# jyf588/transformer-inertial-poser

Measured on AMD Instinct MI355X. Metric: IMU frames/sec (whole node), seq_len=40 batch=256/GPU, higher is better.
Workload: dtype f32

## Files before the change

### include/tip_hip.h

```cpp
#ifndef TIP_HIP_H
#define TIP_HIP_H

#include <stddef.h>
#include <stdint.h>

#ifdef __cplusplus
extern "C" {
#endif

#define TIP_ABI_VERSION 5

#define TIP_API __attribute__((visibility("default")))

typedef struct tip_handle tip_handle;
typedef void* tip_stream_t;

typedef struct tip_config {
    int32_t input_size_imu;
    int32_t size_s;
    int32_t rnn_hid_size;
    int32_t tf_hid_size;
    int32_t tf_in_dim;
    int32_t n_heads;
    int32_t tf_layers;
// ... 19 lines not shown

#define TIP_PLAN_AUTO    0
#define TIP_PLAN_GENERAL 1
#define TIP_PLAN_FUSED   2
#define TIP_PLAN_FUSED2  4
#define TIP_PLAN_FUSEDH  6
#define TIP_PLAN_LATENCY 3

#define TIP_PLAN_FUSED1S 10

#define TIP_OPT_PLAN        1
#define TIP_OPT_PROFILE     2
#define TIP_OPT_RNN_CLUSTER 3
#define TIP_RNN_CLUSTER_ROWS4 0x44
#define TIP_OPT_FAULT_INJECT 4

#define TIP_OPT_FUSE_HEAD 5

#define TIP_OPT_AUTO_DEMOTE 7
#define TIP_OPT_DEMOTED     8
#define TIP_OPT_NO_FLOW    10
#define TIP_OPT_HANDOFF_KIND 11
#define TIP_OPT_NO_ROUND_LAUNCH 12
#define TIP_OPT_F1S_PARTS   9

TIP_API int tip_abi_version(void);
TIP_API int tip_create(const tip_config* cfg, tip_handle** out);
TIP_API void tip_destroy(tip_handle* h);
TIP_API const char* tip_strerror(int status);
TIP_API const char* tip_last_hip_error(const tip_handle* h);
TIP_API int tip_set_option(tip_handle* h, int option, int value);
TIP_API int tip_get_option(const tip_handle* h, int option, int* value);

TIP_API int tip_num_tensors(const tip_handle* h);
TIP_API int tip_tensor_info(const tip_handle* h, int i, const char** name, int* rows, int* cols );
TIP_API int tip_packed_bytes(const tip_handle* h, size_t* bytes);
TIP_API int tip_pack_weights(const tip_handle* h, const float* const* host_tensors, int n, void* packed_host_out, size_t bytes);
TIP_API int tip_pack_weights_device(const tip_handle* h, const float* const* tensors, int n, void* packed_dev, size_t bytes,
                            tip_stream_t stream);
TIP_API int tip_attach_packed(tip_handle* h, const void* packed_device, size_t bytes);

TIP_API int tip_workspace_bytes(const tip_handle* h, int B, int T, size_t* bytes);
TIP_API int tip_max_batch(const tip_handle* h, int T, int fp64, int* max_batch);
TIP_API int tip_forward(tip_handle* h, const float* x_imu, const float* x_s, float* y, int B, int T, int flags,
                const float* keep_mask, float keep_scale, void* workspace, size_t workspace_bytes,
                tip_stream_t stream);
// ... 283 lines not shown
```

### transformer-inertial-poser_amd/csrc/tip_abi.hip

```cpp
#include <math.h>
#include <string.h>

#include <new>

#include <mutex>
#include "tip_internal.h"
#include <atomic>
#include <chrono>

using namespace tip;

namespace {

const char* kStatusText[] = {
    "ok",
    "invalid argument",
    "unsupported configuration",
    "not ready: no packed weights attached",
    "workspace too small or misaligned",
    "HIP runtime error",
    "no HIP device",
    "allocation failure",
    "an inter-workgroup hand-off wait gave up in an earlier launch (outputs of that launch are NaN-poisoned); tip_check(h, 1) clears",
};

size_t align_up(size_t x, size_t a) { return (x + a - 1) / a * a; }

void build_tensor_table(tip_handle* h) {
    const Dims& d = h->d;
    auto add = [&](const std::string& n, int r, int cdim) {
        h->tensor_names.push_back(n);
// ... 89 lines not shown
        stop = pr.second;
    }
    ~StageScope() {
        if (stop) (void)hipEventRecord(stop, s);
    }
};

}

static hipError_t linear_gemm(const float* P, const tip::PackedLinear& p, const float* A, int lda, const float* res, int ldres,
                              float* C, int ldc, int M, int flags, hipStream_t s) {
    auto al16 = [](const void* q, int ld) { return (reinterpret_cast<uintptr_t>(q) & 15) == 0 && (ld & 3) == 0; };
    if (p.f_off && tip::pgemm_shape_ok(M, p.N, p.K) && al16(P + p.b_off, 0) && al16(C, ldc) && (!(flags & 2) || al16(res, ldres)))
        return tip::launch_pgemm(A, lda, P + p.f_off, (size_t)p.N * p.K, P + p.b_off, res, ldres, C, ldc, M, p.N, p.K, flags, s);
    return tip::launch_gemm(A, lda, P + p.w_off, p.Kpad, P + p.b_off, res, ldres, C, ldc, M, p.N, p.Npad, flags, s);
}

namespace tip {
namespace {
struct DevSerialState {
    std::mutex mu;
    hipStream_t last = nullptr;
    bool have = false;
    hipEvent_t ev = nullptr;
};
DevSerialState g_serial[kMaxDevices];
}

CoopSerial::CoopSerial(int device, hipStream_t s)
    : dev(device >= 0 && device < kMaxDevices ? device : tip_cur_device()), stream(s), capturing(stream_is_capturing(s)), status(hipSuccess) {
    DevSerialState& st = g_serial[dev];
    st.mu.lock();
    if (capturing) return;
    if (st.have && st.last != s && st.ev) status = hipStreamWaitEvent(s, st.ev, 0);
}

CoopSerial::~CoopSerial() {
    DevSerialState& st = g_serial[dev];
    if (!capturing) {
        if (!st.ev && hipEventCreateWithFlags(&st.ev, hipEventDisableTiming) != hipSuccess) {
            (void)hipGetLastError();
            st.ev = nullptr;
        }
        if (st.ev) (void)hipEventRecord(st.ev, stream);
        st.last = stream;
        st.have = true;
    }
    st.mu.unlock();
}
}

extern "C" {

int tip_abi_version(void) { return TIP_ABI_VERSION; }

const char* tip_strerror(int status) {
    const int i = -status;
    if (i < 0 || i >= (int)(sizeof(kStatusText) / sizeof(kStatusText[0]))) return "unknown status";
    return kStatusText[i];
}

int tip_create(const tip_config* cfg, tip_handle** out) {
    if (!cfg || !out) return TIP_ERR_INVALID_ARG;
    *out = nullptr;
    Dims d{};
    d.n_imu_total = cfg->input_size_imu + (cfg->with_acc_sum ? 18 : 0);
    d.S = cfg->size_s;
    d.In = d.n_imu_total + d.S;
    d.InPad = round_up(d.In, kGemmBK);
    d.D = cfg->tf_in_dim;
    d.H = cfg->n_heads;
// ... 42 lines not shown
            if (hipHostGetDevicePointer(&dp, hp, 0) == hipSuccess && dp) {
                h->err_host = static_cast<unsigned*>(hp);
                h->err_dev = static_cast<unsigned*>(dp);
            } else {
                (void)hipHostFree(hp);
            }
        }
        (void)hipGetLastError();
    } else {
        (void)hipGetLastError();
    }
    *out = h;
    return TIP_OK;
}

void tip_destroy(tip_handle* h) {
    if (!h) return;
    for (auto& t : h->timers)
        for (auto& pr : t.pairs) {
            (void)hipEventDestroy(pr.first);
            (void)hipEventDestroy(pr.second);
        }
    if (h->err_host) (void)hipHostFree(h->err_host);
    delete h;
}

const char* tip_last_hip_error(const tip_handle* h) { return h ? h->last_hip_error.c_str() : ""; }

int tip_set_option(tip_handle* h, int option, int value) {
    if (!h) return TIP_ERR_INVALID_ARG;
    switch (option) {
        case TIP_OPT_PLAN:
            if (value < TIP_PLAN_AUTO || value > TIP_PLAN_FUSED1S || value == 9 ) return TIP_ERR_INVALID_ARG;
            if (value == 5 || value == 7 || value == 8) return TIP_ERR_UNSUPPORTED_CONFIG;
            h->plan = value;
            return TIP_OK;
        case TIP_OPT_PROFILE:
            if (value < 0 || value > 3) return TIP_ERR_INVALID_ARG;
            h->profile = value;
            for (auto& t : h->timers) t.used = 0;
            return TIP_OK;
        case TIP_OPT_RNN_CLUSTER:
            if (!(value == 0 || value == 1 || value == 2 || value == 4 || value == 8 || value == 16 || value == 32 || value == TIP_RNN_CLUSTER_ROWS4))
                return TIP_ERR_INVALID_ARG;
            h->rnn_cluster = value;
            return TIP_OK;
// ... 5 lines not shown
            if (value < 0 || value > 1) return TIP_ERR_INVALID_ARG;
            h->fuse_head = value;
            return TIP_OK;
        case TIP_OPT_AUTO_DEMOTE:
            if (value < 0 || value > 1) return TIP_ERR_INVALID_ARG;
            h->auto_demote = value;
            return TIP_OK;
        case TIP_OPT_DEMOTED:
            if (value < 0 || value > 1) return TIP_ERR_INVALID_ARG;
            h->demoted = value;
            return TIP_OK;
        case TIP_OPT_F1S_PARTS:
            if (value != 0 && value != 2 && value != 4) return TIP_ERR_INVALID_ARG;
            h->f1s_parts = value;
            return TIP_OK;
        case TIP_OPT_NO_FLOW:
            if (value < 0 || value > 1) return TIP_ERR_INVALID_ARG;
            h->no_flow = value;
            return TIP_OK;
        case TIP_OPT_NO_ROUND_LAUNCH:
            if (value < 0 || value > 1) return TIP_ERR_INVALID_ARG;
            h->no_round_launch = value;
            return TIP_OK;
        default: return TIP_ERR_INVALID_ARG;
    }
}

int tip_check(tip_handle* h, int clear) {
    if (!h) return TIP_ERR_INVALID_ARG;
    if (!h->err_host) return TIP_OK;
    volatile unsigned* w = const_cast<volatile unsigned*>(h->err_host);
    const unsigned v = w[0] | w[1];
    if (clear) w[0] = w[1] = 0u;
    return v ? TIP_ERR_HANDOFF : TIP_OK;
}

int tip_get_option(const tip_handle* h, int option, int* value) {
    if (!h || !value) return TIP_ERR_INVALID_ARG;
    switch (option) {
        case TIP_OPT_PLAN: *value = h->plan; return TIP_OK;
        case TIP_OPT_PROFILE: *value = h->profile; return TIP_OK;
        case TIP_OPT_RNN_CLUSTER: *value = h->rnn_cluster; return TIP_OK;
        case TIP_OPT_FAULT_INJECT: *value = h->fault_inject; return TIP_OK;
        case TIP_OPT_FUSE_HEAD: *value = h->fuse_head; return TIP_OK;
        case TIP_OPT_AUTO_DEMOTE: *value = h->auto_demote; return TIP_OK;
        case TIP_OPT_DEMOTED: *value = h->demoted; return TIP_OK;
        case TIP_OPT_F1S_PARTS: *value = h->f1s_parts; return TIP_OK;
        case TIP_OPT_NO_FLOW: *value = h->no_flow; return TIP_OK;
        case TIP_OPT_NO_ROUND_LAUNCH: *value = h->no_round_launch; return TIP_OK;
        case TIP_OPT_HANDOFF_KIND: {
            const volatile unsigned* w = const_cast<const volatile unsigned*>(h->err_host);
            *value = !w ? 0 : w[0] ? 1 : w[1] ? 2 : 0;
            return TIP_OK;
        }
        default: return TIP_ERR_INVALID_ARG;
    }
}

int tip_num_tensors(const tip_handle* h) { return h ? (int)h->tensor_names.size() : TIP_ERR_INVALID_ARG; }

int tip_tensor_info(const tip_handle* h, int i, const char** name, int* rows, int* cols) {
    if (!h || i < 0 || i >= (int)h->tensor_names.size()) return TIP_ERR_INVALID_ARG;
    if (name) *name = h->tensor_names[i].c_str();
    if (rows) *rows = h->tensor_shapes[i].first;
    if (cols) *cols = h->tensor_shapes[i].second;
    return TIP_OK;
}

int tip_packed_bytes(const tip_handle* h, size_t* bytes) {
    if (!h || !bytes) return TIP_ERR_INVALID_ARG;
    *bytes = h->lay.total_floats * sizeof(float);
    return TIP_OK;
// ... 104 lines not shown
    bool rnn_done = false, head_done = false;
    bool round_launch = false;
};

#define TIP_TRY(expr, what)                                     \
    do {                                                        \
        const hipError_t e_ = (expr);                           \
        if (e_ != hipSuccess) return fail_hip(q.h, e_, what);   \
    } while (0)
#define TIP_STAGE(name, expr)              \
    do {                                   \
        StageScope stage_(q.h, q.s, name); \
        TIP_TRY(expr, name);               \
    } while (0)

static int launch_round(LaunchSeq& q, const float* x_imu, const float* x_s, const float* mask, float* ih, float* hall) {
    tip_handle* h = q.h;
    const Dims& d = h->d;
    const float* P = h->packed_dev;
    const PackedLayout& L = h->lay;
    const bool last_only = (q.flags & TIP_FWD_LAST_ROW_ONLY) != 0;
    const int head = q.T == 40 && measure_switches().head_ksplit ? (last_only ? 2 : 1) : 0;
    StageScope sc(h, q.s, "fused_encoder");
    const hipError_t e = launch_forward_round(d, P + L.fused_off, x_imu, x_s, mask, q.keep_scale, ih, hall,
                                              reinterpret_cast<unsigned*>(q.W0 + q.ws.flags), P + L.whh_frag_off, P + L.out_frag_off,
                                              P + L.out_lin.b_off, q.y, q.n, q.T, head, q.cus, h->guard(), q.s);
    if (e == hipErrorCooperativeLaunchTooLarge || e == hipErrorInvalidValue) {
        (void)hipGetLastError();
        return 0;
    }
    if (e != hipSuccess) return fail_hip(h, e, "forward_round");
    q.ih_done = q.hall_armed = q.rnn_done = true;
    q.head_done = head != 0;
    return 1;
}

static int run_encoder(LaunchSeq& q, const SchedPart& p, int off) {
    tip_handle* h = q.h;
    const Dims& d = h->d;
    const float* P = h->packed_dev;
    const PackedLayout& L = h->lay;
    hipStream_t s = q.s;
    const int B = p.count, T = q.T, cus = q.cus, M = B * T;
    const size_t row_i = (size_t)T * d.n_imu_total, row_s = (size_t)T * d.S, row_r = (size_t)T * d.R;
    const float* x_imu = q.x_imu + off * row_i;
    const float* x_s = q.x_s + off * row_s;
    const float* mask = q.mask ? q.mask + off * row_s : nullptr;
    const float keep_scale = q.keep_scale;
    float* xa = q.W0 + q.ws.xa;
// ... 289 lines not shown
```

### transformer-inertial-poser_amd/csrc/tip_fused_h.h

```cpp
#pragma once
#include "tip_internal.h"
#include "tip_attention.h"
#include "tip_layernorm.h"

namespace tip {

typedef float f32x4 __attribute__((ext_vector_type(4)));

namespace fz {
constexpr int D = 256, H = 16, DH = 16, F = 1024, RP = 48, RB = 3, TMAX = 40, R = 512;
constexpr int KIN = 224;
constexpr int LDX = D + 8;
constexpr int LDC = 128 + 4;
constexpr int LDV = RP + 4;
constexpr int LDU = KIN + 8;
constexpr int X_FLOATS = RP * LDX;
constexpr int C_FLOATS = 2 * RP * LDC + 128 * LDV;
constexpr int LDS_BYTES = (X_FLOATS + C_FLOATS) * 4;
constexpr int THREADS = 512;
constexpr size_t IN_W = 0;
constexpr size_t IN_B = IN_W + (size_t)D * KIN;
constexpr size_t LAYER0 = IN_B + D;
constexpr size_t QKV_W = 0;
constexpr size_t QKV_B = QKV_W + (size_t)3 * D * D;
// ... 201 lines not shown
}

__device__ __forceinline__ f32x4 tail_gather_v(const f32x4& a0, const f32x4& a1, int lg) {
    f32x4 o;
#pragma unroll
    for (int e = 0; e < 4; ++e) {
        float x = a0[e], y = a1[e];
        swap16(x, y);
        float s = x + y, t = s;
        swap32(s, t);
        o[e] = s + t;
    }
    return lg < 2 ? o : (f32x4){0.f, 0.f, 0.f, 0.f};
}

extern __device__ unsigned long long g_fh_trace[64];
extern __device__ unsigned long long g_fh_wg[2 * 1024];
#define FH_STAMP(slot) do { if (TRACE && blockIdx.x == 0 && tid == 0 && (layer == 1 || (slot) < 4 || (slot) >= 40)) g_fh_trace[slot] = __builtin_amdgcn_s_memtime(); } while (0)

struct FhGridStride {
    static constexpr int kAux = 0;
    __device__ __forceinline__ int first() const { return blockIdx.x; }
    __device__ __forceinline__ int stride() const { return gridDim.x; }
    __device__ __forceinline__ void published(int, int) const {}
};

template <bool TRACE, bool TR, bool LIVE, class Ctl>
__device__ __forceinline__ void fused_encoder_h_body(
    const float* __restrict__ wts, const float* __restrict__ x_imu, const float* __restrict__ x_s, const float* __restrict__ keep_mask, float keep_scale, float* __restrict__ xout, float* __restrict__ ih_out,
    unsigned* __restrict__ hall_sentinel, int B, int T, int NI, int S, int L, int wbytes, int ih_off_b, const FusedEncArgs<LIVE>& tr, Ctl ctl) {
#include "tip_fused_h_body.inc"
}

}
```

### transformer-inertial-poser_amd/csrc/tip_fused_h_body.inc

```
    using namespace fz;
    using namespace fzh;
    extern __shared__ __attribute__((aligned(16))) float smem[];
    float* X = smem;
    float* C = smem + X_FLOATS;
    const int tid = threadIdx.x, lane = tid & 63;
    const int wave = __builtin_amdgcn_readfirstlane(tid >> 6);
    const int l15 = lane & 15, lg = lane >> 4;
    const __amdgpu_buffer_rsrc_t rsrc = __builtin_amdgcn_make_buffer_rsrc(const_cast<float*>(wts), 0, wbytes, 0x00020000);
    const int voff = lane * 16;
    auto am = [&](int ld) { return l15 * ld + lg * 4; };
    auto at = [&](int ld) { return (TAIL0 + (lane & 3)) * ld + lg * 4; };
    constexpr bool DR = TR || LIVE;
    const LiveArgs lv = live_args_of(tr);
    unsigned long long dseed = tr.seed, sseed = 0;
    if (LIVE) {
        sseed = lv.state_seed;
        if (lv.seeds) { dseed = lv.seeds[0]; sseed = lv.seeds[1]; }
    }
    const unsigned mkey = LIVE && lv.mthresh ? tip_drop_key_s(sseed, kStateMaskSite) : 0u;

    for (int i = tid; i < 8 * LDX; i += THREADS) X[TMAX * LDX + i] = 0.f;

    for (int win = ctl.first(); win < B; win += ctl.stride()) {
        WRing<3> g_qkv;
// ... 319 lines not shown
            const int lo = opaque(lane), l15o = lo & 15, lgo = lo >> 4;
            float bvs[4];
            f32x4 bv4s[4];
#pragma unroll
            for (int n = 0; n < 4; ++n) {
                bvs[n] = wts[ih_off_b / 4 + R * D + (wave * 4 + n) * 16 + l15o];
                bv4s[n] = *reinterpret_cast<const f32x4*>(wts + ih_off_b / 4 + R * D + (wave * 4 + n) * 16 + lgo * 4);
            }
#pragma unroll
            for (int n = 0; n < 4; ++n) {
                const int col = (wave * 4 + n) * 16 + l15o;
#pragma unroll
                for (int r = 0; r < RBM; ++r) {
                    const int row = r * 16 + l15o;
                    __builtin_amdgcn_raw_buffer_store_b128(__builtin_bit_cast(u32x4, acc[r][n] + bv4s[n]), io_rs, (row * R + (wave * 4 + n) * 16 + lgo * 4) * 4, 0, Ctl::kAux);
                }
#pragma unroll
                for (int r = 0; r < RBT; ++r) {
                    const float v = tail_reduce(acct[r][n], lg) + bvs[n];
                    const int row = TAIL0 + 4 * r + lgo;
                    __builtin_amdgcn_raw_buffer_store_b32(__float_as_uint(v), io_rs, (row * R + col) * 4, 0, Ctl::kAux);
                }
            }
        }
        if (hall_sentinel) {
            if constexpr (Ctl::kAux != 0) {
                const __amdgpu_buffer_rsrc_t hs_rs = __builtin_amdgcn_make_buffer_rsrc(hall_sentinel + (size_t)win * T * R, 0, T * R * 4, 0x00020000);
                const u32x4 ones = {0xFFFFFFFFu, 0xFFFFFFFFu, 0xFFFFFFFFu, 0xFFFFFFFFu};
                for (int i = opaque(tid); i < T * (R / 4); i += THREADS) __builtin_amdgcn_raw_buffer_store_b128(ones, hs_rs, i * 16, 0, Ctl::kAux);
            } else {
            uint4* hp = reinterpret_cast<uint4*>(hall_sentinel + (size_t)win * T * R);
            for (int i = opaque(tid); i < T * (R / 4); i += THREADS) hp[i] = make_uint4(0xFFFFFFFFu, 0xFFFFFFFFu, 0xFFFFFFFFu, 0xFFFFFFFFu);
            }
        }
        if (xout) {
            float* out = xout + (size_t)win * T * D;
            for (int i = tid; i < T * (D / 4); i += THREADS) {
                const int r = i / (D / 4), c4 = i - r * (D / 4);
                *reinterpret_cast<float4*>(out + (size_t)r * D + c4 * 4) = *reinterpret_cast<const float4*>(X + r * LDX + c4 * 4);
            }
        }
        __syncthreads();
        { const int layer = -1; FH_STAMP(41); }
        if (TRACE && tid == 0 && blockIdx.x < 1024) g_fh_wg[2 * blockIdx.x + 1] = __builtin_amdgcn_s_memrealtime();
        ctl.published(win, tid);
    }
// ... 1 lines not shown
```

### transformer-inertial-poser_amd/csrc/tip_rnn_rows4.h

```cpp
#pragma once
#include "tip_internal.h"
#include "tip_layernorm.h"

namespace tip {

typedef float f32x4 __attribute__((ext_vector_type(4)));
typedef unsigned int u32x4 __attribute__((ext_vector_type(4)));

constexpr unsigned kRnnSentinel = 0xFFFFFFFFu;
constexpr int kQ4Rows = 4, kQ4Cluster = 4, kQ4Tiles = 4, kQ4LD = 512 + 16;

struct RnnFromMemory {
    static constexpr bool kRound = false;
    static constexpr int kIhAux = 0;
    __device__ __forceinline__ bool inputs_ready(int, unsigned, const Guard&) const { return true; }
    __device__ __forceinline__ void member_lost(int) const {}
};

extern __device__ unsigned long long g_rnn_trace[2048];

}
```

### transformer-inertial-poser_amd/csrc/tip_rnn_rows4_body.inc

```
    constexpr int R = 512, KB = R / 16, CLUSTER = 32 / WAVES, LD = kQ4LD;
    constexpr int THREADS = WAVES * 64, PL = 8 / WAVES;
    static_assert(WAVES == 8 || WAVES == 4, "cluster of 4 or 8 members");
    extern __shared__ __attribute__((aligned(16))) float smem[];
    const int tid = threadIdx.x, lane = tid & 63;
    const int wave = __builtin_amdgcn_readfirstlane(tid >> 6);
    const int l15 = lane & 15, lg = lane >> 4;
    if (TRACE && blockIdx.x == 0 && tid == 0) g_rnn_trace[3] = __builtin_amdgcn_s_memtime();
    const int cid = (blockIdx.x >> 3) % CLUSTER, group = (blockIdx.x & 7) + 8 * ((blockIdx.x >> 3) / CLUSTER);
    if (group >= ngroups) return;
    const int nb = cid * WAVES + wave;
    const __amdgpu_buffer_rsrc_t hrs = __builtin_amdgcn_make_buffer_rsrc(hall, 0, hall_bytes, 0x00020000);
    const __amdgpu_buffer_rsrc_t irs = __builtin_amdgcn_make_buffer_rsrc(const_cast<float*>(ih), 0, hall_bytes, 0x00020000);
    const __amdgpu_buffer_rsrc_t grs = __builtin_amdgcn_make_buffer_rsrc(const_cast<float*>(BWD ? gate : ih), 0, hall_bytes, 0x00020000);
    const bool dead = (gd.fault & 2) && group == 0 && cid == 1;
    if (dead) return;
    const unsigned spin_big = guard_spin_limit(gd.fault, 1u << 22), spin_pull = guard_spin_limit(gd.fault, 1u << 20);

    const int prow = tid / (THREADS / 4), pcol = (tid % (THREADS / 4)) * (4 * PL);
    const int tpg = (ntiles + ngroups - 1) / ngroups;
    const unsigned rowbytes = (unsigned)T * R * 4;
    int vpull[NT], vout[NT];
    auto set_tiles = [&](int q0) {
#pragma unroll
        for (int n = 0; n < NT; ++n) {
// ... 8 lines not shown
        const int so = te_ * (R * 4);
#pragma unroll
        for (int n = 0; n < NT; ++n) {
            ihn[n] = __builtin_bit_cast(float, __builtin_amdgcn_raw_buffer_load_b32(irs, vout[n], so, Ctl::kIhAux));
            gn[n] = BWD ? __builtin_bit_cast(float, __builtin_amdgcn_raw_buffer_load_b32(grs, vout[n], so, 0)) : 0.f;
        }
    };
    u32x4 pfv[NT];
    auto touch_rows = [&](int te_) {
        const int so = te_ * (R * 4);
#pragma unroll
        for (int n = 0; n < NT; ++n) pfv[n] = __builtin_amdgcn_raw_buffer_load_b128(hrs, vpull[n], so, 16);
    };
    auto retire_touch = [&]() {
#pragma unroll
        for (int n = 0; n < NT; ++n) asm volatile("" :: "v"(pfv[n]));
    };
    set_tiles(0);
    if constexpr (!Ctl::kRound) {
    request_inputs(BWD ? T - 1 : 0);
    touch_rows(BWD ? T - 1 : 0);
    }
    float4 wreg[KB];
    {
        const float4* wf = reinterpret_cast<const float4*>(whh_frag) + (size_t)nb * KB * 64 + lane;
#pragma unroll
        for (int k = 0; k < KB; ++k) wreg[k] = wf[(size_t)k * 64];
    }
    __shared__ int s_same_xcd;
    if (tid == 0 && dead) s_same_xcd = 0;
    if (tid == 0 && !dead) {
        unsigned xcc;
        asm volatile("s_getreg_b32 %0, hwreg(HW_REG_XCC_ID)" : "=s"(xcc));
        xcc &= 0xf;
        const unsigned mine = (etag << 5) | (xcc + 1u);
        __hip_atomic_store(flags + group * CLUSTER + cid, mine, __ATOMIC_RELAXED, __HIP_MEMORY_SCOPE_AGENT);
        bool same = true;
        for (int m = 0; m < CLUSTER; ++m) {
            unsigned v = 0;
            bool here = false;
            for (unsigned spins = 0; spins < spin_big; ++spins) {
                v = __hip_atomic_load(flags + group * CLUSTER + m, __ATOMIC_RELAXED, __HIP_MEMORY_SCOPE_AGENT);
                here = (v >> 5) == etag && (v & 31u) != 0u;
                if (here) break;
                __builtin_amdgcn_s_sleep(1);
            }
            if (!here) note_spin_timeout(gd.err);
            if constexpr (Ctl::kRound) if (!here) ctl.member_lost(m);
            same &= (v == mine);
        }
        if constexpr (Ctl::kRound)
            s_same_xcd = ((same && !(gd.fault & 8)) ? 1 : 0) | (ctl.inputs_ready(group, spin_big, gd) ? 0 : 2);
        else
        s_same_xcd = (same && !(gd.fault & 8)) ? 1 : 0;
    }
    __syncthreads();
    bool same_xcd_;
    if constexpr (Ctl::kRound) same_xcd_ = (s_same_xcd & 1) != 0;
    else same_xcd_ = s_same_xcd != 0;
    const bool same_xcd = same_xcd_;
    if (TRACE && blockIdx.x == 0 && tid == 0) {
        asm volatile("s_waitcnt vmcnt(0)" ::: "memory");
        g_rnn_trace[7] = __builtin_amdgcn_s_memtime();
    }
    const int aoff = (lane & 3) * LD + lg * 4;
    const int lds_w = prow * LD + pcol;
    bool poisoned = false;
    if constexpr (Ctl::kRound) {
        request_inputs(0);
        touch_rows(0);
        if (s_same_xcd & 2) {
            poisoned = true;
#pragma unroll
            for (int n = 0; n < NT; ++n) ihn[n] = __uint_as_float(kPoisonBits);
        }
    }
    if (TRACE && tid == 0 && blockIdx.x < 512) {
        unsigned hwid, xccid;
        asm volatile("s_getreg_b32 %0, hwreg(HW_REG_HW_ID)" : "=s"(hwid));
        asm volatile("s_getreg_b32 %0, hwreg(HW_REG_XCC_ID)" : "=s"(xccid));
        g_rnn_trace[1024 + blockIdx.x] = (unsigned long long)hwid | ((unsigned long long)(xccid & 0xf) << 32);
    }

    u32x4 pv[PL];
#pragma unroll
    for (int i = 0; i < PL; ++i) pv[i] = (u32x4){kRnnSentinel, kRnnSentinel, kRnnSentinel, kRnnSentinel};
    auto run_steps = [&](auto same_tag) {
        constexpr bool SAME_XCD = decltype(same_tag)::value;
        for (int q0 = dead ? tpg : 0; q0 < tpg; q0 += NT) {
            if (q0 > 0) {
                set_tiles(q0);
// ... 122 lines not shown
                    float a1 = p[1], a3 = p[3];
                    swap32(a1, a3);
                    float k1 = a1 + a3;
                    swap16(k0, k1);
                    const float acc = k0 + k1;
                    if (TRACE && !(abl & 128) && n == 0 && blockIdx.x == 0 && tid == 0 && t < 64) {
                        asm volatile("" :: "v"(acc));
                        g_rnn_trace[t * 4 + 1] = __builtin_amdgcn_s_memtime();
                    }
                    if (TRACE && (abl & 128) && ((abl >> 8) & 7) == 2 && n == 0 && blockIdx.x == 0 && tid == 0 && t < 64) {
                        asm volatile("" :: "v"(c0[0]), "v"(c1[0]), "v"(c2[0]), "v"(c3[0]));
                        g_rnn_trace[t * 4 + 1] = __builtin_amdgcn_s_memtime();
                    }
#ifdef TIP_MEASURE
                    float hv = BWD ? (acc + ihv[n]) * (1.0f - gv[n] * gv[n])
                                   : ((abl & 32) ? fminf(fmaxf(acc + ihv[n], -1.0f), 1.0f) : tip_tanh(acc + ihv[n]));
#else
                    float hv = BWD ? (acc + ihv[n]) * (1.0f - gv[n] * gv[n]) : tip_tanh(acc + ihv[n]);
#endif
                    if (hv != hv) hv = __uint_as_float(kPoisonBits);
                    __builtin_amdgcn_raw_buffer_store_b32(__float_as_uint(hv), hrs, vout[n], so_out, SAME_XCD ? 0 : 16);
                }
                if (TRACE && blockIdx.x == 0 && tid == 0 && t < 64) g_rnn_trace[t * 4 + 2] = __builtin_amdgcn_s_memtime();
            }
            retire_touch();
            __syncthreads();
        }
    };
    if (same_xcd) run_steps(std::true_type{});
    else run_steps(std::false_type{});
    if (T >= 2 && tid == 0 && !dead) __hip_atomic_store(flags + group * CLUSTER + cid, 0u, __ATOMIC_RELAXED, __HIP_MEMORY_SCOPE_AGENT);
```

### transformer-inertial-poser_amd/csrc/tip_round.hip

```cpp
#include "tip_fused_h.h"
#include "tip_head.h"
#include "tip_rnn_rows4.h"

namespace tip {

__device__ unsigned g_spin_timeouts_round;
__device__ __forceinline__ void note_spin_timeout(unsigned* err) {
    atomicAdd(&g_spin_timeouts_round, 1u);
    guard_report(err);
}
hipError_t read_spin_timeouts_round(unsigned* out) {
    return hipMemcpyFromSymbol(out, HIP_SYMBOL(g_spin_timeouts_round), sizeof(unsigned));
}

__device__ unsigned long long g_round_wg[5 * 1024];

namespace {

constexpr int kRoundFlag0 = 512;
constexpr int kRoundMaxB = 256;
constexpr int kRoundLds = hd::LDS_BYTES > fz::LDS_BYTES ? hd::LDS_BYTES : fz::LDS_BYTES;
static_assert(2 * kQ4Rows * kQ4LD * (int)sizeof(float) <= kRoundLds, "the recurrence's tile buffers fit the other phases' LDS");

__device__ __forceinline__ unsigned round_flag_value(unsigned etag) { return (etag << 1) | 1u; }

struct RoundEncCtl {
    static constexpr int kAux = 16;
    int B;
    unsigned* wflags;
    unsigned etag;
    __device__ __forceinline__ int first() const { return blockIdx.x; }
    __device__ __forceinline__ int stride() const { return B; }
    __device__ __forceinline__ void published(int win, int tid) const {
        asm volatile("s_waitcnt vmcnt(0)" ::: "memory");
        __syncthreads();
        if (tid == 0) __hip_atomic_store(wflags + win, round_flag_value(etag), __ATOMIC_RELAXED, __HIP_MEMORY_SCOPE_AGENT);
    }
};

struct RoundRnnCtl {
    static constexpr bool kRound = true;
    static constexpr int kIhAux = 16;
    int B;
    const unsigned* wflags;
    unsigned etag;
    unsigned* lost;
    __device__ __forceinline__ void member_lost(int m) const { *lost |= 1u << m; }
    __device__ __forceinline__ bool inputs_ready(int group, unsigned spin_limit, const Guard& gd) const {
        bool ok = true;
        for (int m = 0; m < kQ4Rows; ++m) {
            const int w = group * kQ4Rows + m;
            if (w >= B) break;
            bool here = false;
            for (unsigned spins = 0; spins < spin_limit; ++spins) {
                here = __hip_atomic_load(wflags + w, __ATOMIC_RELAXED, __HIP_MEMORY_SCOPE_AGENT) == round_flag_value(etag);
                if (here) break;
                __builtin_amdgcn_s_sleep(4);
            }
            if (!here) {
                note_spin_timeout(gd.err);
                ok = false;
            }
        }
        return ok;
    }
};

template <class Ctl>
__device__ __forceinline__ void rnn_rows4_round_body(const float* __restrict__ ih, const float* __restrict__ whh_frag, float* __restrict__ hall,
                                                     unsigned* __restrict__ flags, int B, int T, int ntiles, int hall_bytes,
// ... 38 lines not shown
};

}

struct RoundArgs {
    const float* wts;
    const float* x_imu;
    const float* x_s;
    const float* keep_mask;
    float keep_scale;
    float* ih;
    float* hall;
    unsigned* flags;
    const float* whh_frag;
    const float* out_frag;
    const float* out_bias;
    float* y;
    int B, T, NI, S, L, wbytes, ih_off_b, hall_bytes, ntiles;
    int head;
    unsigned etag;
    Guard gd;
};

template <bool TRACE>
__global__ __launch_bounds__(fz::THREADS) void forward_round_kernel(RoundArgs a) {
    constexpr int CLUSTER = kQ4Cluster;
    const int tid = threadIdx.x;
    const int cid = (blockIdx.x >> 3) % CLUSTER, group = (blockIdx.x & 7) + 8 * ((blockIdx.x >> 3) / CLUSTER);
    if (TRACE && tid == 0 && blockIdx.x < 1024) {
        unsigned xcc;
        asm volatile("s_getreg_b32 %0, hwreg(HW_REG_XCC_ID)" : "=s"(xcc));
        g_round_wg[4096 + blockIdx.x] = xcc & 0xf;
        g_round_wg[4 * blockIdx.x] = __builtin_amdgcn_s_memrealtime();
    }
    if ((a.gd.fault & 2) && group == 0 && cid == 1) return;
    unsigned* wflags = a.flags + kRoundFlag0;
    __shared__ unsigned s_lost;
    if (tid == 0) s_lost = 0u;

    if ((int)blockIdx.x < a.B)
        fused_encoder_h_body<false, false, false>(a.wts, a.x_imu, a.x_s, a.keep_mask, a.keep_scale, nullptr, a.ih, reinterpret_cast<unsigned*>(a.hall),
                                                  a.B, a.T, a.NI, a.S, a.L, a.wbytes, a.ih_off_b, FusedTrain{}, RoundEncCtl{a.B, wflags, a.etag});
    if (TRACE && tid == 0 && blockIdx.x < 1024) g_round_wg[4 * blockIdx.x + 1] = __builtin_amdgcn_s_memrealtime();
    __syncthreads();

    rnn_rows4_round_body(a.ih, a.whh_frag, a.hall, a.flags, a.B, a.T, a.ntiles, a.hall_bytes, nullptr, a.gd, a.etag, 0, a.ntiles,
                         RoundRnnCtl{a.B, wflags, a.etag, &s_lost});
    if (TRACE && tid == 0 && blockIdx.x < 1024) g_round_wg[4 * blockIdx.x + 2] = __builtin_amdgcn_s_memrealtime();

    const int w = group * kQ4Rows + cid;
    const __amdgpu_buffer_rsrc_t hrs = __builtin_amdgcn_make_buffer_rsrc(a.hall, 0, a.hall_bytes, 0x00020000);
    const unsigned spin_limit = guard_spin_limit(a.gd.fault, 1u << 20);
    __syncthreads();
    if (a.head == 1) {
        if (w < a.B)
            head_ksplit_body<0, false, 16>(a.hall, 2048u, (unsigned)a.hall_bytes, a.out_frag, a.out_bias, a.y, a.S, a.B * a.T, a.S, a.B,
                                           RoundHdCtl{w, a.B, hrs, w, 1, a.T, spin_limit, a.gd.err, true});
    } else if (a.head == 2) {
        if (cid == 0 && group < a.ntiles) {
            const int nw = a.B - group * kQ4Rows < kQ4Rows ? a.B - group * kQ4Rows : kQ4Rows;
            const RoundHdCtl hc{group, a.ntiles, hrs, group * kQ4Rows, nw, a.T, spin_limit, a.gd.err, false};
            hc.wait_rows();
            head_ksplit_body<2, false, 16>(a.hall + (size_t)(a.T - 1) * 512, (unsigned)a.T * 2048u,
                                           (unsigned)a.hall_bytes - (unsigned)(a.T - 1) * 2048u, a.out_frag, a.out_bias, a.y, a.S, a.B, a.S,
                                           a.ntiles, hc);
        }
    }
    if (a.head != 0 && group < a.ntiles && s_lost != 0u) {
        for (int m = 0; m < kQ4Rows; ++m) {
            const int wl = group * kQ4Rows + m;
            if (!((s_lost >> m) & 1u) || wl >= a.B) continue;
            const int n = a.head == 1 ? a.T * a.S : a.S;
            float* yl = a.y + (size_t)wl * n;
            for (int i = tid; i < n; i += fz::THREADS) yl[i] = __uint_as_float(kPoisonBits);
        }
    }
    if (w < a.B && tid < 64) {
        const bool done = a.head == 1 ? true : round_wait_last_row(hrs, w, a.T, spin_limit);
        if (a.head == 1 || done) {
            if (tid == 0) __hip_atomic_store(wflags + w, 0u, __ATOMIC_RELAXED, __HIP_MEMORY_SCOPE_AGENT);
        } else if (tid == 0) {
            note_spin_timeout(a.gd.err);
        }
    }
    if (TRACE && tid == 0 && blockIdx.x < 1024) g_round_wg[4 * blockIdx.x + 3] = __builtin_amdgcn_s_memrealtime();
}
#undef FH_STAMP

bool round_launch_shape(const Dims& d, int B, int T, int num_cus) {
    const int grid = (((B + kQ4Rows - 1) / kQ4Rows + 7) / 8) * 8 * kQ4Cluster;
    return fused_supported(d, T) && fused_has_rnn_ih(d) && d.R == 512 && d.S >= 129 && d.S <= 131 && B >= 1 && B <= kRoundMaxB &&
           grid <= num_cus && (long long)(B + 7) * T * 512 * 4 <= 0x7fffffffLL;
}

hipError_t launch_forward_round(const Dims& d, const float* fused_w, const float* x_imu, const float* x_s, const float* keep_mask,
                                float keep_scale, float* ih, float* hall, unsigned* flags, const float* whh_frag, const float* out_frag,
                                const float* out_bias, float* y, int B, int T, int head, int num_cus, const Guard& gd, hipStream_t s) {
    if (!round_launch_shape(d, B, T, num_cus) || (head != 0 && T != 40) || head < 0 || head > 2) return hipErrorInvalidValue;
    if (hipError_t e = dynamic_lds<forward_round_kernel<false>, forward_round_kernel<true>>(kRoundLds)) return e;
    const int ntiles = (B + kQ4Rows - 1) / kQ4Rows;
    const int grid = (ntiles + 7) / 8 * 8 * kQ4Cluster;
    static PerDeviceInt occ_dev; int& occ = occ_dev.cur();
    if (hipError_t ce = check_coresident(forward_round_kernel<false>, fz::THREADS, (size_t)kRoundLds, grid, num_cus, &occ)) return ce;
    RoundArgs a{fused_w, x_imu, x_s, keep_mask, keep_scale, ih, hall, flags, whh_frag, out_frag, out_bias, y, B, T, d.n_imu_total, d.S, d.L,
                (int)(fused_packed_floats(d) * 4), (int)((fz::LAYER0 + (size_t)d.L * fz::LAYER_FLOATS) * 4), (int)((long long)B * T * 512 * 4),
                ntiles, head, next_rnn_launch_tag(), gd};
    if (measure_switches().fusedh_trace)
        hipLaunchKernelGGL(forward_round_kernel<true>, dim3(grid), dim3(fz::THREADS), kRoundLds, s, a);
    else
        hipLaunchKernelGGL(forward_round_kernel<false>, dim3(grid), dim3(fz::THREADS), kRoundLds, s, a);
    return hipGetLastError();
}

hipError_t read_round_wg(unsigned long long* out, int n) {
    return hipMemcpyFromSymbol(out, HIP_SYMBOL(g_round_wg), sizeof(unsigned long long) * n);
}

}
```

### transformer-inertial-poser_amd/lib.py

```python
from __future__ import annotations

import contextlib
import ctypes
import os
import subprocess
from typing import List, Optional, Tuple

import torch

_HERE = os.path.dirname(os.path.abspath(__file__))
CSRC = os.path.join(_HERE, "csrc")
MEASURE = os.environ.get("TIP_LIB", "") == "measure"
LIB_PATH = os.path.join(CSRC, "libtip_hip_measure.so" if MEASURE else "libtip_hip.so")
if os.environ.get("TIP_LIB", "").endswith(".so"):
    LIB_PATH = os.path.abspath(os.environ["TIP_LIB"])

TIP_FWD_LAST_ROW_ONLY = 0x1
TIP_FWD_KEEP_MASK = 0x2
TIP_PLAN_AUTO, TIP_PLAN_GENERAL, TIP_PLAN_FUSED, TIP_PLAN_LATENCY, TIP_PLAN_FUSED2, TIP_PLAN_FUSEDH = 0, 1, 2, 3, 4, 6
TIP_PLAN_FUSED1S = 10
TIP_SAVED_QKV, TIP_SAVED_ATT, TIP_SAVED_X1, TIP_SAVED_HID, TIP_SAVED_XOUT, TIP_SAVED_HALL = range(6)
TIP_STREAM_FRAME_AUTO = -1
TIP_OPT_PLAN, TIP_OPT_PROFILE, TIP_OPT_RNN_CLUSTER, TIP_OPT_FAULT_INJECT, TIP_OPT_FUSE_HEAD = 1, 2, 3, 4, 5
TIP_OPT_AUTO_DEMOTE, TIP_OPT_DEMOTED, TIP_OPT_F1S_PARTS = 7, 8, 9
TIP_OPT_NO_ROUND_LAUNCH = 12
TIP_OPT_NO_FLOW, TIP_OPT_HANDOFF_KIND = 10, 11
TIP_ABI_VERSION = 5
TIP_RNN_CLUSTER_ROWS4 = 0x44
TIP_ERR_HANDOFF = -8
TIP_ERR_HIP = -5
TIP_ERR_UNSUPPORTED_CONFIG = -2
TIP_LOSS_Q, TIP_LOSS_C, TIP_LOSS_J, TIP_LOSS_STATS = 1, 2, 4, 16
TIP_SENSOR_HEADING, TIP_SENSOR_TPOSE = 1, 2
TIP_RESAMPLE_HOLD, TIP_RESAMPLE_SLERP = 0, 1
TIP_RESAMPLE_PREDICTED = 5
TIP_CLOCK_LEAK, TIP_CLOCK_SLEW, TIP_PREDICT_SPAN = 2e-4, 0.5, 2.0

EXPORTS = (
    "tip_abi_version", "tip_create", "tip_destroy", "tip_strerror", "tip_last_hip_error", "tip_set_option",
    "tip_get_option", "tip_num_tensors", "tip_tensor_info", "tip_packed_bytes", "tip_pack_weights",
    "tip_pack_weights_device", "tip_attach_packed", "tip_workspace_bytes", "tip_max_batch", "tip_forward", "tip_forward_dropout", "tip_draw_keep_mask", "tip_forward_f64_bytes", "tip_forward_f64", "tip_forward_count", "tip_profile_read",
    "tip_spin_timeouts", "tip_check", "tip_stream_state_bytes", "tip_stream_reset", "tip_stream_window_len", "tip_stream_ingest", "tip_stream_consume",
    "tip_reuse_cache_bytes", "tip_reuse_reset", "tip_forward_reuse", "tip_stream_frame_counter_offset", "tip_stream_ingest_newest",
    "tip_forward_rows", "tip_stream_attach", "tip_stream_detach", "tip_stream_ingest_staggered", "tip_stream_consume_staggered",
    "tip_stream_ingest_mapped", "tip_stream_consume_mapped", "tip_stream_reset_shaped", "tip_stream_history_override",
    "tip_forward_live", "tip_seeds_next",
    "tip_stream_state_bytes_w", "tip_stream_window_len_w", "tip_stream_reset_w", "tip_stream_ingest_w", "tip_stream_consume_w",
    "tip_stream_attach_w", "tip_stream_detach_w", "tip_stream_ingest_staggered_w", "tip_stream_consume_staggered_w",
# ... 438 lines not shown
```

Measured before the change: 415,800.

## Add first-look RNN entry handshake in round kernel and lazy cross-stream serialization

```diff
diff --git a/include/tip_hip.h b/include/tip_hip.h
--- a/include/tip_hip.h
+++ b/include/tip_hip.h
@@ -65,6 +65,7 @@
 #define TIP_OPT_NO_FLOW    10
 #define TIP_OPT_HANDOFF_KIND 11
 #define TIP_OPT_NO_ROUND_LAUNCH 12
+#define TIP_OPT_ROUND_ENTRY 13
 #define TIP_OPT_F1S_PARTS   9
 
 TIP_API int tip_abi_version(void);
diff --git a/transformer-inertial-poser_amd/csrc/tip_abi.hip b/transformer-inertial-poser_amd/csrc/tip_abi.hip
--- a/transformer-inertial-poser_amd/csrc/tip_abi.hip
+++ b/transformer-inertial-poser_amd/csrc/tip_abi.hip
@@ -5,8 +5,10 @@
 
 #include <mutex>
 #include "tip_internal.h"
+#include "tip_rnn_rows4.h"
 #include <atomic>
 #include <chrono>
+#include <unordered_map>
 
 using namespace tip;
 
@@ -142,6 +144,7 @@
     std::mutex mu;
     hipStream_t last = nullptr;
     bool have = false;
+    bool several = false;
     hipEvent_t ev = nullptr;
 };
 DevSerialState g_serial[kMaxDevices];
@@ -152,21 +155,44 @@
     DevSerialState& st = g_serial[dev];
     st.mu.lock();
     if (capturing) return;
-    if (st.have && st.last != s && st.ev) status = hipStreamWaitEvent(s, st.ev, 0);
+    if (!st.have || st.last == s) return;
+    if (!st.several) {
+        int cur = -1;
+        const bool move = hipGetDevice(&cur) == hipSuccess && cur != dev;
+        if (move) status = hipSetDevice(dev);
+        if (status == hipSuccess) status = hipDeviceSynchronize();
+        if (move) (void)hipSetDevice(cur);
+        st.several = true;
+        return;
+    }
+    if (st.ev) status = hipStreamWaitEvent(s, st.ev, 0);
 }
 
 CoopSerial::~CoopSerial() {
     DevSerialState& st = g_serial[dev];
     if (!capturing) {
-        if (!st.ev && hipEventCreateWithFlags(&st.ev, hipEventDisableTiming) != hipSuccess) {
-            (void)hipGetLastError();
-            st.ev = nullptr;
-        }
-        if (st.ev) (void)hipEventRecord(st.ev, stream);
+        if (st.several) {
+            if (!st.ev && hipEventCreateWithFlags(&st.ev, hipEventDisableTiming) != hipSuccess) {
+                (void)hipGetLastError();
+                st.ev = nullptr;
+            }
+            if (st.ev) (void)hipEventRecord(st.ev, stream);
+        }
         st.last = stream;
         st.have = true;
     }
     st.mu.unlock();
+}
+}
+
+namespace {
+std::mutex g_round_entry_mu;
+std::unordered_map<const tip_handle*, int> g_round_entry;
+int round_entry_of(const tip_handle* h) {
+    std::lock_guard<std::mutex> lk(g_round_entry_mu);
+    if (g_round_entry.empty()) return tip::kRoundEntryDefault;
+    const auto it = g_round_entry.find(h);
+    return it == g_round_entry.end() ? tip::kRoundEntryDefault : it->second;
 }
 }
 
@@ -255,6 +281,10 @@
             (void)hipEventDestroy(pr.second);
         }
     if (h->err_host) (void)hipHostFree(h->err_host);
+    {
+        std::lock_guard<std::mutex> lk(g_round_entry_mu);
+        g_round_entry.erase(h);
+    }
     delete h;
 }
 
@@ -306,6 +336,12 @@
             if (value < 0 || value > 1) return TIP_ERR_INVALID_ARG;
             h->no_round_launch = value;
             return TIP_OK;
+        case TIP_OPT_ROUND_ENTRY: {
+            if (value < 0 || value > 1) return TIP_ERR_INVALID_ARG;
+            std::lock_guard<std::mutex> lk(g_round_entry_mu);
+            g_round_entry[h] = value;
+            return TIP_OK;
+        }
         default: return TIP_ERR_INVALID_ARG;
     }
 }
@@ -332,6 +368,7 @@
         case TIP_OPT_F1S_PARTS: *value = h->f1s_parts; return TIP_OK;
         case TIP_OPT_NO_FLOW: *value = h->no_flow; return TIP_OK;
         case TIP_OPT_NO_ROUND_LAUNCH: *value = h->no_round_launch; return TIP_OK;
+        case TIP_OPT_ROUND_ENTRY: *value = round_entry_of(h); return TIP_OK;
         case TIP_OPT_HANDOFF_KIND: {
             const volatile unsigned* w = const_cast<const volatile unsigned*>(h->err_host);
             *value = !w ? 0 : w[0] ? 1 : w[1] ? 2 : 0;
@@ -482,9 +519,11 @@
     const bool last_only = (q.flags & TIP_FWD_LAST_ROW_ONLY) != 0;
     const int head = q.T == 40 && measure_switches().head_ksplit ? (last_only ? 2 : 1) : 0;
     StageScope sc(h, q.s, "fused_encoder");
+    Guard gd = h->guard();
+    gd.fault |= (round_entry_of(h) & 1) << kRoundOrderShift;
     const hipError_t e = launch_forward_round(d, P + L.fused_off, x_imu, x_s, mask, q.keep_scale, ih, hall,
                                               reinterpret_cast<unsigned*>(q.W0 + q.ws.flags), P + L.whh_frag_off, P + L.out_frag_off,
-                                              P + L.out_lin.b_off, q.y, q.n, q.T, head, q.cus, h->guard(), q.s);
+                                              P + L.out_lin.b_off, q.y, q.n, q.T, head, q.cus, gd, q.s);
     if (e == hipErrorCooperativeLaunchTooLarge || e == hipErrorInvalidValue) {
         (void)hipGetLastError();
         return 0;
diff --git a/transformer-inertial-poser_amd/csrc/tip_fused_h.h b/transformer-inertial-poser_amd/csrc/tip_fused_h.h
--- a/transformer-inertial-poser_amd/csrc/tip_fused_h.h
+++ b/transformer-inertial-poser_amd/csrc/tip_fused_h.h
@@ -247,6 +247,7 @@
     static constexpr int kAux = 0;
     __device__ __forceinline__ int first() const { return blockIdx.x; }
     __device__ __forceinline__ int stride() const { return gridDim.x; }
+    __device__ __forceinline__ void ih_stored() const {}
     __device__ __forceinline__ void published(int, int) const {}
 };
 
diff --git a/transformer-inertial-poser_amd/csrc/tip_fused_h_body.inc b/transformer-inertial-poser_amd/csrc/tip_fused_h_body.inc
--- a/transformer-inertial-poser_amd/csrc/tip_fused_h_body.inc
+++ b/transformer-inertial-poser_amd/csrc/tip_fused_h_body.inc
@@ -365,6 +365,7 @@
                     __builtin_amdgcn_raw_buffer_store_b32(__float_as_uint(v), io_rs, (row * R + col) * 4, 0, Ctl::kAux);
                 }
             }
+            ctl.ih_stored();
         }
         if (hall_sentinel) {
             if constexpr (Ctl::kAux != 0) {
diff --git a/transformer-inertial-poser_amd/csrc/tip_rnn_rows4.h b/transformer-inertial-poser_amd/csrc/tip_rnn_rows4.h
--- a/transformer-inertial-poser_amd/csrc/tip_rnn_rows4.h
+++ b/transformer-inertial-poser_amd/csrc/tip_rnn_rows4.h
@@ -9,12 +9,18 @@
 
 constexpr unsigned kRnnSentinel = 0xFFFFFFFFu;
 constexpr int kQ4Rows = 4, kQ4Cluster = 4, kQ4Tiles = 4, kQ4LD = 512 + 16;
+constexpr int kRoundOrderShift = 8;
+constexpr int kRoundEntryDefault = 0;
 
 struct RnnFromMemory {
     static constexpr bool kRound = false;
+    static constexpr bool kFirstLook = false;
     static constexpr int kIhAux = 0;
     __device__ __forceinline__ bool inputs_ready(int, unsigned, const Guard&) const { return true; }
     __device__ __forceinline__ void member_lost(int) const {}
+    __device__ __forceinline__ const unsigned* window_flag(int, int, bool& in_range) const { in_range = false; return nullptr; }
+    __device__ __forceinline__ bool flag_ok(unsigned) const { return true; }
+    __device__ __forceinline__ void stamp(int) const {}
 };
 
 extern __device__ unsigned long long g_rnn_trace[2048];
diff --git a/transformer-inertial-poser_amd/csrc/tip_rnn_rows4_body.inc b/transformer-inertial-poser_amd/csrc/tip_rnn_rows4_body.inc
--- a/transformer-inertial-poser_amd/csrc/tip_rnn_rows4_body.inc
+++ b/transformer-inertial-poser_amd/csrc/tip_rnn_rows4_body.inc
@@ -54,12 +54,13 @@
     touch_rows(BWD ? T - 1 : 0);
     }
     float4 wreg[KB];
-    {
+    if constexpr (!Ctl::kFirstLook) {
         const float4* wf = reinterpret_cast<const float4*>(whh_frag) + (size_t)nb * KB * 64 + lane;
 #pragma unroll
         for (int k = 0; k < KB; ++k) wreg[k] = wf[(size_t)k * 64];
     }
     __shared__ int s_same_xcd;
+    if constexpr (!Ctl::kFirstLook) {
     if (tid == 0 && dead) s_same_xcd = 0;
     if (tid == 0 && !dead) {
         unsigned xcc;
@@ -81,14 +82,18 @@
             if constexpr (Ctl::kRound) if (!here) ctl.member_lost(m);
             same &= (v == mine);
         }
-        if constexpr (Ctl::kRound)
+        if constexpr (Ctl::kRound) {
+            ctl.stamp(5);
             s_same_xcd = ((same && !(gd.fault & 8)) ? 1 : 0) | (ctl.inputs_ready(group, spin_big, gd) ? 0 : 2);
-        else
+            ctl.stamp(6);
+        } else
         s_same_xcd = (same && !(gd.fault & 8)) ? 1 : 0;
     }
     __syncthreads();
+    }
     bool same_xcd_;
-    if constexpr (Ctl::kRound) same_xcd_ = (s_same_xcd & 1) != 0;
+    if constexpr (Ctl::kFirstLook) same_xcd_ = false;
+    else if constexpr (Ctl::kRound) same_xcd_ = (s_same_xcd & 1) != 0;
     else same_xcd_ = s_same_xcd != 0;
     const bool same_xcd = same_xcd_;
     if (TRACE && blockIdx.x == 0 && tid == 0) {
@@ -98,7 +103,7 @@
     const int aoff = (lane & 3) * LD + lg * 4;
     const int lds_w = prow * LD + pcol;
     bool poisoned = false;
-    if constexpr (Ctl::kRound) {
+    if constexpr (Ctl::kRound && !Ctl::kFirstLook) {
         request_inputs(0);
         touch_rows(0);
         if (s_same_xcd & 2) {
@@ -267,11 +272,98 @@
                     __builtin_amdgcn_raw_buffer_store_b32(__float_as_uint(hv), hrs, vout[n], so_out, SAME_XCD ? 0 : 16);
                 }
                 if (TRACE && blockIdx.x == 0 && tid == 0 && t < 64) g_rnn_trace[t * 4 + 2] = __builtin_amdgcn_s_memtime();
+                if constexpr (Ctl::kRound) if (t == 0) ctl.stamp(7);
             }
             retire_touch();
             __syncthreads();
         }
     };
+    if constexpr (Ctl::kFirstLook) {
+        __shared__ int s_entry[2];
+        constexpr unsigned XMASK = (1u << CLUSTER) - 1u;
+        unsigned mine = 0u, v = 0u;
+        bool watch = false, is_x = false, here = true;
+        const unsigned* pw = flags;
+        if (wave == 0) {
+            unsigned xcc;
+            asm volatile("s_getreg_b32 %0, hwreg(HW_REG_XCC_ID)" : "=s"(xcc));
+            xcc &= 0xf;
+            mine = (etag << 5) | (xcc + 1u);
+            if (lane == 0) __hip_atomic_store(flags + group * CLUSTER + cid, mine, __ATOMIC_RELAXED, __HIP_MEMORY_SCOPE_AGENT);
+            is_x = lane < CLUSTER;
+            if (is_x) {
+                pw = flags + group * CLUSTER + lane;
+                watch = lane != cid;
+                v = mine;
+            } else if (lane < CLUSTER + kQ4Rows) {
+                pw = ctl.window_flag(group, lane - CLUSTER, watch);
+            }
+        }
+        auto look = [&]() {
+            if (watch) {
+                v = __hip_atomic_load(pw, __ATOMIC_RELAXED, __HIP_MEMORY_SCOPE_AGENT);
+                here = is_x ? ((v >> 5) == etag && (v & 31u) != 0u) : ctl.flag_ok(v);
+            }
+        };
+        if (wave == 0) {
+            here = !watch;
+            look();
+            const bool all = __builtin_amdgcn_ballot_w64(!here) == 0;
+            const bool same = __builtin_amdgcn_ballot_w64(is_x && v != mine) == 0;
+            if (lane == 0) s_entry[0] = all ? (4 | ((same && !(gd.fault & 8)) ? 1 : 0)) : 0;
+        }
+        __syncthreads();
+        const int e0 = __builtin_amdgcn_readfirstlane(s_entry[0]);
+        auto load_whh = [&]() {
+            const float4* wf = reinterpret_cast<const float4*>(whh_frag) + (size_t)nb * KB * 64 + lane;
+#pragma unroll
+            for (int k = 0; k < KB; ++k) wreg[k] = wf[(size_t)k * 64];
+        };
+        if (e0 & 4) {
+            ctl.stamp(6);
+            request_inputs(0);
+            touch_rows(0);
+            load_whh();
+            ctl.stamp(5);
+            if (e0 & 1) run_steps(std::true_type{});
+            else run_steps(std::false_type{});
+        } else {
+            load_whh();
+            if (wave == 0) {
+                bool x_seen = false;
+                for (unsigned spins = 0; spins < spin_big; ++spins) {
+                    if (!here) look();
+                    const unsigned pend = (unsigned)__builtin_amdgcn_ballot_w64(!here);
+                    if (!x_seen && !(pend & XMASK)) { x_seen = true; ctl.stamp(5); }
+                    if (pend == 0u) break;
+                    if (pend & XMASK) __builtin_amdgcn_s_sleep(1);
+                    else __builtin_amdgcn_s_sleep(4);
+                }
+                ctl.stamp(6);
+                if (!here) note_spin_timeout(gd.err);
+                const unsigned lostm = (unsigned)__builtin_amdgcn_ballot_w64(is_x && !here);
+                const bool in_lost = __builtin_amdgcn_ballot_w64(!is_x && !here) != 0;
+                const bool same = __builtin_amdgcn_ballot_w64(is_x && v != mine) == 0;
+                if (lane == 0) {
+                    for (int m = 0; m < CLUSTER; ++m)
+                        if ((lostm >> m) & 1u) ctl.member_lost(m);
+                    s_entry[1] = ((same && !(gd.fault & 8)) ? 1 : 0) | (in_lost ? 2 : 0);
+                }
+            }
+            __syncthreads();
+            const int e1 = __builtin_amdgcn_readfirstlane(s_entry[1]);
+            request_inputs(0);
+            touch_rows(0);
+            if (e1 & 2) {
+                poisoned = true;
+#pragma unroll
+                for (int n = 0; n < NT; ++n) ihn[n] = __uint_as_float(kPoisonBits);
+            }
+            if (e1 & 1) run_steps(std::true_type{});
+            else run_steps(std::false_type{});
+        }
+    } else {
     if (same_xcd) run_steps(std::true_type{});
     else run_steps(std::false_type{});
+    }
     if (T >= 2 && tid == 0 && !dead) __hip_atomic_store(flags + group * CLUSTER + cid, 0u, __ATOMIC_RELAXED, __HIP_MEMORY_SCOPE_AGENT);
diff --git a/transformer-inertial-poser_amd/csrc/tip_round.hip b/transformer-inertial-poser_amd/csrc/tip_round.hip
--- a/transformer-inertial-poser_amd/csrc/tip_round.hip
+++ b/transformer-inertial-poser_amd/csrc/tip_round.hip
@@ -14,6 +14,11 @@
 }
 
 __device__ unsigned long long g_round_wg[5 * 1024];
+template <bool TRACE>
+__device__ __forceinline__ void round_stamp(int k) {
+    if constexpr (TRACE)
+        if (threadIdx.x == 0 && blockIdx.x < 512) g_round_wg[8 * blockIdx.x + k] = __builtin_amdgcn_s_memrealtime();
+}
 
 namespace {
 
@@ -24,6 +29,7 @@
 
 __device__ __forceinline__ unsigned round_flag_value(unsigned etag) { return (etag << 1) | 1u; }
 
+template <bool TRACE>
 struct RoundEncCtl {
     static constexpr int kAux = 16;
     int B;
@@ -31,6 +37,7 @@
     unsigned etag;
     __device__ __forceinline__ int first() const { return blockIdx.x; }
     __device__ __forceinline__ int stride() const { return B; }
+    __device__ __forceinline__ void ih_stored() const { round_stamp<TRACE>(4); }
     __device__ __forceinline__ void published(int win, int tid) const {
         asm volatile("s_waitcnt vmcnt(0)" ::: "memory");
         __syncthreads();
@@ -38,14 +45,23 @@
     }
 };
 
+template <bool TRACE, bool FIRSTLOOK>
 struct RoundRnnCtl {
     static constexpr bool kRound = true;
+    static constexpr bool kFirstLook = FIRSTLOOK;
     static constexpr int kIhAux = 16;
     int B;
     const unsigned* wflags;
     unsigned etag;
     unsigned* lost;
     __device__ __forceinline__ void member_lost(int m) const { *lost |= 1u << m; }
+    __device__ __forceinline__ void stamp(int k) const { round_stamp<TRACE>(k); }
+    __device__ __forceinline__ const unsigned* window_flag(int group, int m, bool& in_range) const {
+        const int w = group * kQ4Rows + m;
+        in_range = w < B;
+        return wflags + (w < B ? w : B - 1);
+    }
+    __device__ __forceinline__ bool flag_ok(unsigned v) const { return v == round_flag_value(etag); }
     __device__ __forceinline__ bool inputs_ready(int group, unsigned spin_limit, const Guard& gd) const {
         bool ok = true;
         for (int m = 0; m < kQ4Rows; ++m) {
@@ -130,17 +146,17 @@
     Guard gd;
 };
 
-template <bool TRACE>
+template <bool TRACE, int ORDER>
 __global__ __launch_bounds__(fz::THREADS) void forward_round_kernel(RoundArgs a) {
     constexpr int CLUSTER = kQ4Cluster;
     const int tid = threadIdx.x;
     const int cid = (blockIdx.x >> 3) % CLUSTER, group = (blockIdx.x & 7) + 8 * ((blockIdx.x >> 3) / CLUSTER);
-    if (TRACE && tid == 0 && blockIdx.x < 1024) {
+    if (TRACE && tid == 0 && blockIdx.x < 512) {
         unsigned xcc;
         asm volatile("s_getreg_b32 %0, hwreg(HW_REG_XCC_ID)" : "=s"(xcc));
         g_round_wg[4096 + blockIdx.x] = xcc & 0xf;
-        g_round_wg[4 * blockIdx.x] = __builtin_amdgcn_s_memrealtime();
-    }
+    }
+    round_stamp<TRACE>(0);
     if ((a.gd.fault & 2) && group == 0 && cid == 1) return;
     unsigned* wflags = a.flags + kRoundFlag0;
     __shared__ unsigned s_lost;
@@ -148,13 +164,14 @@
 
     if ((int)blockIdx.x < a.B)
         fused_encoder_h_body<false, false, false>(a.wts, a.x_imu, a.x_s, a.keep_mask, a.keep_scale, nullptr, a.ih, reinterpret_cast<unsigned*>(a.hall),
-                                                  a.B, a.T, a.NI, a.S, a.L, a.wbytes, a.ih_off_b, FusedTrain{}, RoundEncCtl{a.B, wflags, a.etag});
-    if (TRACE && tid == 0 && blockIdx.x < 1024) g_round_wg[4 * blockIdx.x + 1] = __builtin_amdgcn_s_memrealtime();
+                                                  a.B, a.T, a.NI, a.S, a.L, a.wbytes, a.ih_off_b, FusedTrain{},
+                                                  RoundEncCtl<TRACE>{a.B, wflags, a.etag});
+    round_stamp<TRACE>(1);
     __syncthreads();
 
     rnn_rows4_round_body(a.ih, a.whh_frag, a.hall, a.flags, a.B, a.T, a.ntiles, a.hall_bytes, nullptr, a.gd, a.etag, 0, a.ntiles,
-                         RoundRnnCtl{a.B, wflags, a.etag, &s_lost});
-    if (TRACE && tid == 0 && blockIdx.x < 1024) g_round_wg[4 * blockIdx.x + 2] = __builtin_amdgcn_s_memrealtime();
+                         RoundRnnCtl<TRACE, !(ORDER & 1)>{a.B, wflags, a.etag, &s_lost});
+    round_stamp<TRACE>(2);
 
     const int w = group * kQ4Rows + cid;
     const __amdgpu_buffer_rsrc_t hrs = __builtin_amdgcn_make_buffer_rsrc(a.hall, 0, a.hall_bytes, 0x00020000);
@@ -191,7 +208,7 @@
             note_spin_timeout(a.gd.err);
         }
     }
-    if (TRACE && tid == 0 && blockIdx.x < 1024) g_round_wg[4 * blockIdx.x + 3] = __builtin_amdgcn_s_memrealtime();
+    round_stamp<TRACE>(3);
 }
 #undef FH_STAMP
 
@@ -205,18 +222,23 @@
                                 float keep_scale, float* ih, float* hall, unsigned* flags, const float* whh_frag, const float* out_frag,
                                 const float* out_bias, float* y, int B, int T, int head, int num_cus, const Guard& gd, hipStream_t s) {
     if (!round_launch_shape(d, B, T, num_cus) || (head != 0 && T != 40) || head < 0 || head > 2) return hipErrorInvalidValue;
-    if (hipError_t e = dynamic_lds<forward_round_kernel<false>, forward_round_kernel<true>>(kRoundLds)) return e;
+    if (hipError_t e = dynamic_lds<forward_round_kernel<false, 0>, forward_round_kernel<false, 1>, forward_round_kernel<true, 0>,
+                                   forward_round_kernel<true, 1>>(kRoundLds))
+        return e;
     const int ntiles = (B + kQ4Rows - 1) / kQ4Rows;
     const int grid = (ntiles + 7) / 8 * 8 * kQ4Cluster;
     static PerDeviceInt occ_dev; int& occ = occ_dev.cur();
-    if (hipError_t ce = check_coresident(forward_round_kernel<false>, fz::THREADS, (size_t)kRoundLds, grid, num_cus, &occ)) return ce;
+    if (hipError_t ce = check_coresident(forward_round_kernel<false, 0>, fz::THREADS, (size_t)kRoundLds, grid, num_cus, &occ)) return ce;
+    const int order = (gd.fault >> kRoundOrderShift) & 1;
+    Guard kgd = gd;
+    kgd.fault &= (1 << kRoundOrderShift) - 1;
     RoundArgs a{fused_w, x_imu, x_s, keep_mask, keep_scale, ih, hall, flags, whh_frag, out_frag, out_bias, y, B, T, d.n_imu_total, d.S, d.L,
                 (int)(fused_packed_floats(d) * 4), (int)((fz::LAYER0 + (size_t)d.L * fz::LAYER_FLOATS) * 4), (int)((long long)B * T * 512 * 4),
-                ntiles, head, next_rnn_launch_tag(), gd};
-    if (measure_switches().fusedh_trace)
-        hipLaunchKernelGGL(forward_round_kernel<true>, dim3(grid), dim3(fz::THREADS), kRoundLds, s, a);
-    else
-        hipLaunchKernelGGL(forward_round_kernel<false>, dim3(grid), dim3(fz::THREADS), kRoundLds, s, a);
+                ntiles, head, next_rnn_launch_tag(), kgd};
+    const bool trace = measure_switches().fusedh_trace;
+    auto launch = [&](auto kernel) { hipLaunchKernelGGL(kernel, dim3(grid), dim3(fz::THREADS), kRoundLds, s, a); };
+    if (order == 0) trace ? launch(forward_round_kernel<true, 0>) : launch(forward_round_kernel<false, 0>);
+    else trace ? launch(forward_round_kernel<true, 1>) : launch(forward_round_kernel<false, 1>);
     return hipGetLastError();
 }
 
diff --git a/transformer-inertial-poser_amd/lib.py b/transformer-inertial-poser_amd/lib.py
--- a/transformer-inertial-poser_amd/lib.py
+++ b/transformer-inertial-poser_amd/lib.py
@@ -24,6 +24,7 @@
 TIP_OPT_PLAN, TIP_OPT_PROFILE, TIP_OPT_RNN_CLUSTER, TIP_OPT_FAULT_INJECT, TIP_OPT_FUSE_HEAD = 1, 2, 3, 4, 5
 TIP_OPT_AUTO_DEMOTE, TIP_OPT_DEMOTED, TIP_OPT_F1S_PARTS = 7, 8, 9
 TIP_OPT_NO_ROUND_LAUNCH = 12
+TIP_OPT_ROUND_ENTRY = 13
 TIP_OPT_NO_FLOW, TIP_OPT_HANDOFF_KIND = 10, 11
 TIP_ABI_VERSION = 5
 TIP_RNN_CLUSTER_ROWS4 = 0x44
```

Result: no change. 419,100 (median of 6 runs) (+0.8%).
